# pagmerek/frave

Hardware: AMD Instinct MI355X
Metric: Mpixels/s encode (transform+quant) at 4096x4096 (higher is better)
Workload: dtype u8->i32

## Files before the change

### frave_amd/csrc/geometry.cpp

```cpp
#include "geometry.hpp"

#include <algorithm>
#include <climits>
#include <cstdlib>
#include <cstring>
#include <deque>

namespace fri {

namespace {

constexpr Int2 kLiterals[11] = {{0, 1}, {-1, 1}, {2, 0}, {-3, -1}, {5, -1}, {1, 3}, {-11, -1}, {9, -5}, {13, 7}, {-31, 3}, {5, -17}};

inline Int2 add(Int2 a, Int2 b) { return {a.x + b.x, a.y + b.y}; }
inline Int2 sub(Int2 a, Int2 b) { return {a.x - b.x, a.y - b.y}; }
inline Int2 neg(Int2 a) { return {-a.x, -a.y}; }
inline int floor_div(int a, int b) { return (a >= 0) ? a / b : -((-a + b - 1) / b); }
inline int pos_mod(int a, int m) {
    int r = a % m;
    return r < 0 ? r + m : r;
}

struct LatticeBasis {
    Int2 zl, zmd;
// ... 383 lines not shown
        for (size_t sh = 0; sh < n_wg; sh++) {
            const Tile &first = g.tiles[g.wg_tiles[sh]], &last = g.tiles[g.wg_tiles[sh + 1] - 1];
            g.max_wg_cells = std::max(g.max_wg_cells, last.cell_begin + last.cell_count - first.cell_begin);
            g.max_wg_tiles = std::max(g.max_wg_tiles, g.wg_tiles[sh + 1] - g.wg_tiles[sh]);
        }
    }
    if (tp.strided_shares && n_wg > 1) {
        std::vector<std::vector<int32_t>> dealt(n_wg);
        size_t next = 0;
        for (bool any = true; any && next < T;) {
            any = false;
            for (size_t sh = 0; sh < n_wg && next < T; sh++)
                if (dealt[sh].size() < (size_t)(g.wg_tiles[sh + 1] - g.wg_tiles[sh])) {
                    dealt[sh].push_back((int32_t)next++);
                    any = true;
                }
        }
        std::vector<Tile> tiles2;
        std::vector<TileCell> meta2;
        std::vector<int32_t> cells2;
        tiles2.reserve(T), meta2.reserve(F), cells2.reserve(F);
        g.max_wg_cells = 0;
        for (size_t sh = 0; sh < n_wg; sh++) {
            int32_t share_cells = 0;
            for (int32_t t_old : dealt[sh]) {
                Tile t = g.tiles[t_old];
                const int32_t begin = (int32_t)meta2.size();
                for (int32_t k = 0; k < t.cell_count; k++) {
                    meta2.push_back(g.tile_meta[t.cell_begin + k]);
                    cells2.push_back(g.tile_cells[t.cell_begin + k]);
                }
                t.cell_begin = begin;
                share_cells += t.cell_count;
                tiles2.push_back(t);
            }
            g.max_wg_cells = std::max(g.max_wg_cells, share_cells);
        }
        g.tiles.swap(tiles2);
        g.tile_meta.swap(meta2);
        g.tile_cells.swap(cells2);
    }
    {
        const size_t cells_target = (size_t)(tp.batch_share_tiles > 0 ? tp.batch_share_tiles : 4) * cells_per_tile;
        size_t merge = 1;
        while (merge * (size_t)g.cells_per_wg < cells_target && merge < n_wg) merge++;
        for (size_t sh = 0; sh < n_wg; sh += merge) g.wg_tiles_batch.push_back(g.wg_tiles[sh]);
        g.wg_tiles_batch.push_back(g.wg_tiles[n_wg]);
        for (size_t k = 0; k + 1 < g.wg_tiles_batch.size(); k++) g.max_wg_tiles_batch = std::max(g.max_wg_tiles_batch, g.wg_tiles_batch[k + 1] - g.wg_tiles_batch[k]);
    }
    int pitch = ((max_w * (int)channels + 15 + 15) / 16) * 16;
    while (((pitch / 4) % 32) != 8 && ((pitch / 4) % 32) != 24) pitch += 16;
    g.lds_pitch = pitch;
    g.lds_rows = max_r;
    return "";
}

void build_inverse_lists(Geometry &g, size_t max_bytes) {
    const StaticTables &st = static_tables();
    const int W = (int)g.width, H = (int)g.height, C = (int)g.channels;
    g.inv_lists.clear();
    g.inv_quads.clear();
    g.inv_dwords.clear();
    g.inv_parts.clear();
    g.inv_rect_bytes = 0;
    auto give_up = [&]() {
        g.inv_quads.clear();
        g.inv_dwords.clear();
        g.inv_parts.clear();
    };
    std::vector<InvTileLists> lists(g.tiles.size());
    std::vector<uint16_t> bitmap;
    for (size_t ti = 0; ti < g.tiles.size(); ti++) {
        const Tile &t = g.tiles[ti];
        const int a0 = (t.x_lo * C) & ~15;
        const int rq = ((t.x_lo + t.width_px) * C - 1 - a0) / 16 + 1;
        if (t.n_rows > 256 || rq > 64) return give_up();
        g.inv_rect_bytes = std::max(g.inv_rect_bytes, t.n_rows * rq * 16);
        bitmap.assign((size_t)t.n_rows * rq, 0);
        for (int c = 0; c < t.cell_count; c++) {
            const Int2 cen = g.centers[g.tile_cells[t.cell_begin + c]];
            for (int s2 = 0; s2 < kCell; s2++) {
                const int x = cen.x + st.leaf_off[s2].x, y = cen.y + st.leaf_off[s2].y;
                if (x < 0 || y < 0 || x >= W || y >= H) continue;
                for (int ch = 0; ch < C; ch++) {
                    const int col = x * C + ch - a0;
                    bitmap[(size_t)(y - t.y_lo) * rq + (col >> 4)] |= (uint16_t)(1u << (col & 15));
                }
            }
        }
        lists[ti].quad_begin = (uint32_t)g.inv_quads.size();
        lists[ti].dword_begin = (uint32_t)g.inv_dwords.size();
        lists[ti].part_begin = (uint32_t)g.inv_parts.size();
        for (int r = 0; r < t.n_rows; r++)
            for (int k = 0; k < rq; k++) {
                const uint16_t m = bitmap[(size_t)r * rq + k];
                if (m == 0xFFFFu) {
                    g.inv_quads.push_back((uint16_t)(r << 8 | k));
                } else if (m) {
                    for (int d = 0; d < 4; d++) {
                        const uint32_t nib = (m >> (4 * d)) & 15u;
                        if (nib == 15u)
                            g.inv_dwords.push_back((uint16_t)(r << 8 | (4 * k + d)));
                        else if (nib)
                            g.inv_parts.push_back((uint32_t)(r << 8 | (4 * k + d)) << 4 | nib);
                    }
                }
// ... 11 lines not shown
```

### frave_amd/csrc/k1_forward.hip

```cpp
#include "device_common.hpp"

namespace fri {
namespace {

constexpr int kFwdThreads = 256;
constexpr int kFwdWaves = kFwdThreads / 64;

constexpr int kMaxPairsPerWave = 2;
constexpr int kMaxItemsPerTile = 2 * kMaxPairsPerWave * kFwdWaves;
constexpr int kMaxChunksPerThread = 6;

struct FwdArgs {
    const uint8_t *pixels;
    size_t pixel_stride;
    int32_t *coefs;
    size_t coef_stride;
    const Tile *tiles;
    const TileCell *tile_meta;
    const int32_t *wg_tiles;
    uint32_t n_wg;
    int32_t width, height;
    uint32_t F;
    int32_t pitch;
    int32_t meta_off;
    int32_t buf_bytes;
    uint32_t cpr, cpr_magic;
    int32_t q_identity;
    int32_t ablate;
    unsigned long long *trace;
    unsigned long long *xcd_stat;
    QMatrix q;
};

__device__ __forceinline__ uint32_t pk_low(uint32_t l, uint32_t r, uint32_t x) { return __builtin_amdgcn_lerp(l, r, x >> 15); }
__device__ __forceinline__ void pk_pair(uint32_t l, uint32_t r, int &dA, int &dB, uint32_t &s) {
    s = pk_low(l, r, l - r);
    dA = (int)(l & 0xFFFFu) - (int)(r & 0xFFFFu);
    dB = (int)(l >> 16) - (int)(r >> 16);
}
__device__ __forceinline__ void unpack_x(uint32_t x, int &dA, int &dB) {
    dA = (int)(short)(x & 0xFFFFu);
    dB = (int)(x + 0x8000u) >> 16;
}

template <int J>
__device__ __forceinline__ uint32_t dpp_sibling(uint32_t v) {
    constexpr int ctrl = J == 0 ? 0xB1 : J == 1 ? 0x4E : J == 2 ? 0x141 : 0x140;
    return (uint32_t)__builtin_amdgcn_mov_dpp((int)v, ctrl, 0xF, 0xF, true);
}
template <int J>
__device__ __forceinline__ void pk_cross(int lane, int tz, uint32_t &s, uint32_t &vlow) {
    uint32_t x;
    if constexpr (J < 4) {
        const uint32_t other = dpp_sibling<J>(s);
        x = other - s;
        const uint32_t flip = ((lane >> J) & 1) ? 0u : 0x00010001u;
        s = __builtin_amdgcn_lerp(s, other, (x >> 15) ^ flip);
    } else {
        const uint2v w = J == 4 ? __builtin_amdgcn_permlane16_swap(s, s, false, false) : __builtin_amdgcn_permlane32_swap(s, s, false, false);
        x = w.x - w.y;
        s = pk_low(w.x, w.y, x);
    }
    if (tz == J) vlow = x;
}
template <int J>
__device__ __forceinline__ int xlane_or(int v) {
    if constexpr (J < 4) {
        return v | (int)dpp_sibling<J>((uint32_t)v);
    } else {
        const uint2v w = J == 4 ? __builtin_amdgcn_permlane16_swap((unsigned)v, (unsigned)v, false, false) : __builtin_amdgcn_permlane32_swap((unsigned)v, (unsigned)v, false, false);
        return (int)(w.x | w.y);
    }
}

__device__ __forceinline__ void fwd_wave_pk(const uint32_t (&leaf)[8], int lane, int (&rA)[8], int (&rB)[8]) {
    uint32_t s8[4], s7[2], s;
#pragma unroll
    for (int i = 0; i < 4; i++) pk_pair(leaf[2 * i], leaf[2 * i + 1], rA[i], rB[i], s8[i]);
#pragma unroll
    for (int i = 0; i < 2; i++) pk_pair(s8[2 * i], s8[2 * i + 1], rA[4 + i], rB[4 + i], s7[i]);
    pk_pair(s7[0], s7[1], rA[6], rB[6], s);
    const int tz = lane ? __builtin_ctz(lane) : 6;
    uint32_t vlow = 0;
    pk_cross<0>(lane, tz, s, vlow);
    pk_cross<1>(lane, tz, s, vlow);
    pk_cross<2>(lane, tz, s, vlow);
    pk_cross<3>(lane, tz, s, vlow);
    pk_cross<4>(lane, tz, s, vlow);
    pk_cross<5>(lane, tz, s, vlow);
    if (lane == 0) vlow = s;
    unpack_x((uint32_t)__shfl((int)vlow, low_source_lane(lane)), rA[7], rB[7]);
}

__device__ __forceinline__ uint32_t validity_tree_pk(uint32_t m, int lane) {
    const uint32_t v8 = (m | (m >> 1)) & 0x00550055u;
    const uint32_t v7 = (v8 | (v8 >> 2)) & 0x00110011u;
    int sv = (int)((v7 | (v7 >> 4)) & 0x00010001u);
    const uint32_t v6 = (uint32_t)sv;
    const int tz = lane ? __builtin_ctz(lane) : 6;
    int vlow = 0;
    sv = xlane_or<0>(sv); if (tz == 0) vlow = sv;
    sv = xlane_or<1>(sv); if (tz == 1) vlow = sv;
    sv = xlane_or<2>(sv); if (tz == 2) vlow = sv;
    sv = xlane_or<3>(sv); if (tz == 3) vlow = sv;
    sv = xlane_or<4>(sv); if (tz == 4) vlow = sv;
    sv = xlane_or<5>(sv); if (tz == 5) vlow = sv;
    if (lane == 0) vlow = sv;
    const uint32_t low = (uint32_t)__shfl(vlow, low_source_lane(lane));
    uint32_t out = (v8 & 0x00010001u) | ((v8 >> 1) & 0x00020002u) | ((v8 >> 2) & 0x00040004u) | ((v8 >> 3) & 0x00080008u);
    out |= ((v7 & 0x00010001u) << 4) | ((v7 & 0x00100010u) << 1);
    out |= (v6 << 6) | (low << 7);
    return out;
}

__device__ __forceinline__ int quant_one(int v, int heap_index, const FwdArgs &a) {
    return v == kNone ? v : v / a.q.q[quant_layer(heap_index)];
}

template <int HALF, bool MASKED, bool QID, bool NT, bool C16 = false>
__device__ __forceinline__ void store_item(int32_t *__restrict__ coefs, uint32_t elem_off, int lane, const int (&res)[8], uint32_t valid,
                                           const FwdArgs &a) {
    int v[8];
#pragma unroll
    for (int i = 0; i < 8; i++) {
        v[i] = res[i];
        if (MASKED && !((valid >> (16 * HALF + i)) & 1u)) v[i] = kNone;
    }
    if (!QID) {
#pragma unroll
        for (int i = 0; i < 4; i++) v[i] = quant_one(v[i], 256 + 4 * lane + i, a);
        v[4] = quant_one(v[4], 128 + 2 * lane, a);
        v[5] = quant_one(v[5], 128 + 2 * lane + 1, a);
        v[6] = quant_one(v[6], 64 + lane, a);
        v[7] = quant_one(v[7], lane, a);
    }
    int32_t *out = coefs + elem_off;
    if constexpr (C16) {
        int16_t *o16 = reinterpret_cast<int16_t *>(coefs) + elem_off;
        if (MASKED) {
#pragma unroll
            for (int i = 0; i < 8; i++) v[i] = v[i] == kNone ? 0 : v[i];
        }
        const uint32_t p0 = ((uint32_t)v[0] & 0xFFFFu) | ((uint32_t)v[1] << 16), p1 = ((uint32_t)v[2] & 0xFFFFu) | ((uint32_t)v[3] << 16);
        const uint32_t p2 = ((uint32_t)v[4] & 0xFFFFu) | ((uint32_t)v[5] << 16);
        *reinterpret_cast<i32x2 *>(o16 + 256 + 4 * lane) = i32x2{(int)p0, (int)p1};
        *reinterpret_cast<uint32_t *>(o16 + 128 + 2 * lane) = p2;
        o16[64 + lane] = (int16_t)v[6];
        o16[lane] = (int16_t)v[7];
        return;
    }
    if constexpr (NT) {
        __builtin_nontemporal_store(i32x4{v[0], v[1], v[2], v[3]}, reinterpret_cast<i32x4 *>(out + 256 + 4 * lane));
        __builtin_nontemporal_store(i32x2{v[4], v[5]}, reinterpret_cast<i32x2 *>(out + 128 + 2 * lane));
        __builtin_nontemporal_store(v[6], out + 64 + lane);
        __builtin_nontemporal_store(v[7], out + lane);
    } else {
        *reinterpret_cast<i32x4 *>(out + 256 + 4 * lane) = i32x4{v[0], v[1], v[2], v[3]};
        *reinterpret_cast<i32x2 *>(out + 128 + 2 * lane) = i32x2{v[4], v[5]};
        out[64 + lane] = v[6];
        out[lane] = v[7];
    }
// ... 124 lines not shown
    } else {
#pragma unroll
        for (int k = 0; k < 7; k++) g[k] = 0x80808080u;
    }
}
__device__ __forceinline__ uint32_t rct_leaf(uint32_t x, uint32_t g) { return (x + 0x01800180u - g) & 0x00FF00FFu; }

template <int DELTA>
__device__ __forceinline__ uint32_t shifted_window(uint32_t d0, uint32_t d1, uint32_t d2, uint32_t s) {
    return s + DELTA < 4u ? __builtin_amdgcn_alignbyte(d1, d0, s + DELTA) : __builtin_amdgcn_alignbyte(d2, d1, s + DELTA - 4u);
}
[[maybe_unused]] __device__ __forceinline__ void fetch_windows_ycc(int buf_off, const int (&rb)[3], uint32_t (&r)[7], uint32_t (&g)[7], uint32_t (&b)[7]) {
    const uint32_t b0 = (uint32_t)(buf_off + rb[0]), b1 = (uint32_t)(buf_off + rb[1] - 3), b2 = (uint32_t)(buf_off + rb[2] - 3);
    const LdsDwordPtr p0 = (LdsDwordPtr)(uintptr_t)(b0 & ~3u), p1 = (LdsDwordPtr)(uintptr_t)(b1 & ~3u), p2 = (LdsDwordPtr)(uintptr_t)(b2 & ~3u);
    const uint32_t d00 = p0[0], d01 = p0[1], d02 = p0[2];
    const uint32_t d10 = p1[0], d11 = p1[1], d12 = p1[2], d13 = p1[3];
    const uint32_t d20 = p2[0], d21 = p2[1], d22 = p2[2];
    const uint32_t s0 = b0 & 3u, s1 = b1 & 3u, s2 = b2 & 3u;
    r[0] = __builtin_amdgcn_alignbyte(d01, d00, s0), g[0] = shifted_window<1>(d00, d01, d02, s0), b[0] = shifted_window<2>(d00, d01, d02, s0);
    r[1] = __builtin_amdgcn_alignbyte(d02, d01, s0), g[1] = shifted_window<1>(d01, d02, d02, s0), b[1] = shifted_window<2>(d01, d02, d02, s0);
    r[2] = __builtin_amdgcn_alignbyte(d11, d10, s1), g[2] = shifted_window<1>(d10, d11, d12, s1), b[2] = shifted_window<2>(d10, d11, d12, s1);
    r[3] = __builtin_amdgcn_alignbyte(d12, d11, s1), g[3] = shifted_window<1>(d11, d12, d13, s1), b[3] = shifted_window<2>(d11, d12, d13, s1);
    r[4] = __builtin_amdgcn_alignbyte(d13, d12, s1), g[4] = shifted_window<1>(d12, d13, d13, s1), b[4] = shifted_window<2>(d12, d13, d13, s1);
    r[5] = __builtin_amdgcn_alignbyte(d21, d20, s2), g[5] = shifted_window<1>(d20, d21, d22, s2), b[5] = shifted_window<2>(d20, d21, d22, s2);
    r[6] = __builtin_amdgcn_alignbyte(d22, d21, s2), g[6] = shifted_window<1>(d21, d22, d22, s2), b[6] = shifted_window<2>(d21, d22, d22, s2);
}
struct YccWeights {
    int kr, kg, kb, bias;
};
[[maybe_unused]] __device__ __forceinline__ YccWeights ycc_weights(int plane) {
    if (plane == 0) return {19595, 38470, 7471, 32768};
    if (plane == 1) return {-11059, -21709, 32768, (128 << 16) + 32767};
    return {32768, -27439, -5329, (128 << 16) + 32767};
}
[[maybe_unused]] __device__ __forceinline__ uint32_t ycc_leaf(uint32_t r, uint32_t g, uint32_t b, const YccWeights &wa, const YccWeights &wb) {
    const int va = (__mul24(wa.kr, (int)(r & 0xFFFFu)) + __mul24(wa.kg, (int)(g & 0xFFFFu)) + __mul24(wa.kb, (int)(b & 0xFFFFu)) + wa.bias) >> 16;
    const int vb = (__mul24(wb.kr, (int)(r >> 16)) + __mul24(wb.kg, (int)(g >> 16)) + __mul24(wb.kb, (int)(b >> 16)) + wb.bias) >> 16;
    return (uint32_t)va | ((uint32_t)vb << 16);
}

template <int I>
__device__ __forceinline__ uint32_t pair_bytes(uint32_t a, uint32_t b) {
    return __builtin_amdgcn_perm(b, a, 0x0C000C00u | ((4u + I) << 16) | (unsigned)I);
}

struct ItemAddr {
    int rb[3];
    uint32_t leaf_mask;
    uint32_t elem_off;
};

__device__ __forceinline__ int rct_source(int ch) { return ch == 2 ? 0 : ch + 1; }

template <int C, bool FAST, bool RCT = false, bool YCC = false>
__device__ __forceinline__ ItemAddr item_addr(const FwdArgs &a, const Tile &t, const TileCell *meta, int it, int ldx, int ldy, int lane_rb, int buf_off,
                                               uint32_t sh_base, uint32_t wc16) {
    const int cl = it / C, plane = it - cl * C, ch = YCC ? 0 : RCT ? rct_source(plane) : plane;
    const TileCell m = meta[cl];
    ItemAddr r;
    r.elem_off = ((uint32_t)plane * a.F + (uint32_t)__builtin_amdgcn_readfirstlane(m.cell)) * kCell;
    const int x0 = m.cx + ldx, y0 = m.cy + ldy;
    const int col = __mul24(x0 - t.x_lo, C) + ch;
    if (FAST) {
        const int cell_base = (__builtin_amdgcn_readfirstlane(m.cy) - t.y_lo) * a.pitch + (__builtin_amdgcn_readfirstlane(m.cx) - t.x_lo) * C + ch + (int)(sh_base & 15u);
        r.rb[0] = cell_base + lane_rb + (C == 1 ? buf_off : 0);
        r.rb[1] = r.rb[0] + (C == 1 ? a.pitch - 1 : a.pitch);
        r.rb[2] = r.rb[0] + (C == 1 ? 2 * a.pitch - 1 : 2 * a.pitch);
    } else {
#pragma unroll
        for (int dy = 0; dy < 3; dy++) {
            const int y = y0 + dy;
            const uint32_t sh = (sh_base + __umul24((uint32_t)y & 15u, wc16)) & 15u;
            r.rb[dy] = __mul24(y - t.y_lo, a.pitch) + (int)sh + col + (C == 1 ? buf_off - (dy ? 1 : 0) : 0);
        }
    }
    r.leaf_mask = 0xFFu;
    if (__builtin_amdgcn_readfirstlane(m.interior) == 0) {
        r.leaf_mask = 0;
#pragma unroll
        for (int j = 0; j < 8; j++) {
            const int x = x0 + leaf_dx(j), y = y0 + leaf_dy(j);
            if (x >= 0 && y >= 0 && x < a.width && y < a.height) r.leaf_mask |= 1u << j;
        }
    }
    return r;
}

template <int C, bool EDGE, bool FAST, int NCH, bool QID, bool NT, bool MEASURE = false, bool C16 = false, bool RCT = false, bool YCC = false>
__global__ void __launch_bounds__(kFwdThreads) fwd_transform_quant_kernel(const FwdArgs a) {
    extern __shared__ __attribute__((aligned(16))) uint8_t lds[];
    if (ablate_flags(a.ablate) & 8) return;
    const int tid = threadIdx.x, lane = tid & 63;
    const int wave = __builtin_amdgcn_readfirstlane(tid >> 6);
    const uint32_t wg = xcd_contiguous_share(blockIdx.x, a.n_wg);
    const int tb = a.wg_tiles[wg], te = a.wg_tiles[wg + 1];
    trace_stamp(a.trace, wg, 0, tid);
    const unsigned long long t_entry = a.xcd_stat ? wall_clock64() : 0ull;
    uint8_t *junk = lds + 2 * a.buf_bytes;
    Tile *lds_tiles = reinterpret_cast<Tile *>(junk + 16 * kFwdThreads);
    if (tid < te - tb) lds_tiles[tid] = a.tiles[tb + tid];
    const uint8_t *img = a.pixels + (size_t)blockIdx.y * a.pixel_stride;
    int32_t *coefs = C16 ? reinterpret_cast<int32_t *>(reinterpret_cast<int16_t *>(a.coefs) + (size_t)blockIdx.y * a.coef_stride)
                         : a.coefs + (size_t)blockIdx.y * a.coef_stride;
    const int ldx = lane_dx(lane), ldy = lane_dy(lane);
    const int lane_rb = ldy * a.pitch + ldx * C;
    const uint32_t a16 = (uint32_t)reinterpret_cast<uintptr_t>(img);
    const uint32_t wc = (uint32_t)a.width * C, wc16 = wc & 15u;

    ChunkMap<NCH> cm;
#pragma unroll
    for (int c = 0; c < NCH; c++) {
        const uint32_t i = (uint32_t)tid + (uint32_t)c * kFwdThreads;
        const uint32_t r = a.cpr == 1 ? i : __umulhi(i, a.cpr_magic);
        cm.r[c] = r;
        cm.k16[c] = 16u * (i - r * a.cpr);
        cm.row_off[c] = r * wc;
    }

    u32x4 st[NCH + 1];
    Tile t = a.tiles[tb];
    stage_issue<C, EDGE, FAST, NCH>(a, t, img, tid, cm, st);
    stage_commit<NCH>(a, t, lds, junk, tid, st);
    __syncthreads();
    trace_stamp(a.trace, wg, 1, tid);

    for (int ti = tb; ti < te; ti++) {
        const uint8_t *cur = lds + ((ti - tb) & 1) * a.buf_bytes;
        const int buf_off = (int)(uint32_t)(uintptr_t)(const __attribute__((address_space(3))) uint8_t *)cur;
        uint8_t *nxt = lds + (((ti - tb) & 1) ^ 1) * a.buf_bytes;
        const bool more = ti + 1 < te;
        Tile tn = t;
        if (more) {
            const Tile &l = lds_tiles[ti + 1 - tb];
            tn.x_lo = __builtin_amdgcn_readfirstlane(l.x_lo);
            tn.y_lo = __builtin_amdgcn_readfirstlane(l.y_lo);
            tn.width_px = __builtin_amdgcn_readfirstlane(l.width_px);
            tn.n_rows = __builtin_amdgcn_readfirstlane(l.n_rows);
            tn.cell_begin = __builtin_amdgcn_readfirstlane(l.cell_begin);
            tn.cell_count = __builtin_amdgcn_readfirstlane(l.cell_count);
            stage_issue<C, EDGE, FAST, NCH>(a, tn, img, tid, cm, st);
        }

        if constexpr (C == 1) __builtin_amdgcn_s_setprio(3);
        const TileCell *meta = reinterpret_cast<const TileCell *>(cur + a.meta_off);
        const int n_items = (ablate_flags(a.ablate) & 2) ? 0 : t.cell_count * C;
        const uint32_t sh_base = a16 + (uint32_t)t.x_lo * C;
        int resA[kMaxPairsPerWave][8], resB[kMaxPairsPerWave][8];
        uint32_t offA[kMaxPairsPerWave], offB[kMaxPairsPerWave], valid[kMaxPairsPerWave];
#pragma unroll
        for (int c = 0; c < kMaxPairsPerWave; c++) {
            const int itA = 2 * (wave + kFwdWaves * c);
            offA[c] = offB[c] = 0;
            valid[c] = 0xFFFFFFFFu;
            if (itA < n_items) {
                const int itB = itA + 1 < n_items ? itA + 1 : itA;
                const ItemAddr A = item_addr<C, FAST, RCT, YCC>(a, t, meta, itA, ldx, ldy, lane_rb, buf_off, sh_base, wc16);
                const ItemAddr B = item_addr<C, FAST, RCT, YCC>(a, t, meta, itB, ldx, ldy, lane_rb, buf_off, sh_base, wc16);
                offA[c] = A.elem_off;
                offB[c] = B.elem_off;
                uint32_t leaf[8];
                if constexpr (C == 1) {
                    uint32_t wA[3], wB[3];
                    fetch_windows(A.rb, wA);
                    fetch_windows(B.rb, wB);
                    if ((A.leaf_mask & B.leaf_mask) != 0xFFu) {
                        mask_windows(A.leaf_mask, wA);
                        mask_windows(B.leaf_mask, wB);
                    }
                    leaf[0] = pair_bytes<0>(wA[0], wB[0]);
                    leaf[1] = pair_bytes<1>(wA[1], wB[1]);
                    leaf[2] = pair_bytes<0>(wA[1], wB[1]);
                    leaf[3] = pair_bytes<0>(wA[2], wB[2]);
                    leaf[4] = pair_bytes<2>(wA[0], wB[0]);
                    leaf[5] = pair_bytes<3>(wA[1], wB[1]);
                    leaf[6] = pair_bytes<2>(wA[1], wB[1]);
                    leaf[7] = pair_bytes<2>(wA[2], wB[2]);
                } else if constexpr (YCC) {
                    uint32_t rA[7], gA[7], bA[7], rB[7], gB[7], bB[7];
                    fetch_windows_ycc(buf_off, A.rb, rA, gA, bA);
                    fetch_windows_ycc(buf_off, B.rb, rB, gB, bB);
                    const YccWeights kA = ycc_weights(itA % 3), kB = ycc_weights(itB % 3);
                    leaf[0] = ycc_leaf(pair_bytes<0>(rA[0], rB[0]), pair_bytes<0>(gA[0], gB[0]), pair_bytes<0>(bA[0], bB[0]), kA, kB);
                    leaf[4] = ycc_leaf(pair_bytes<2>(rA[1], rB[1]), pair_bytes<2>(gA[1], gB[1]), pair_bytes<2>(bA[1], bB[1]), kA, kB);
                    leaf[2] = ycc_leaf(pair_bytes<0>(rA[2], rB[2]), pair_bytes<0>(gA[2], gB[2]), pair_bytes<0>(bA[2], bB[2]), kA, kB);
                    leaf[1] = ycc_leaf(pair_bytes<3>(rA[2], rB[2]), pair_bytes<3>(gA[2], gB[2]), pair_bytes<3>(bA[2], bB[2]), kA, kB);
                    leaf[6] = ycc_leaf(pair_bytes<2>(rA[3], rB[3]), pair_bytes<2>(gA[3], gB[3]), pair_bytes<2>(bA[3], bB[3]), kA, kB);
                    leaf[5] = ycc_leaf(pair_bytes<1>(rA[4], rB[4]), pair_bytes<1>(gA[4], gB[4]), pair_bytes<1>(bA[4], bB[4]), kA, kB);
                    leaf[3] = ycc_leaf(pair_bytes<0>(rA[5], rB[5]), pair_bytes<0>(gA[5], gB[5]), pair_bytes<0>(bA[5], bB[5]), kA, kB);
                    leaf[7] = ycc_leaf(pair_bytes<2>(rA[6], rB[6]), pair_bytes<2>(gA[6], gB[6]), pair_bytes<2>(bA[6], bB[6]), kA, kB);
                    if ((A.leaf_mask & B.leaf_mask) != 0xFFu) {
#pragma unroll
                        for (int j = 0; j < 8; j++) {
                            if (!((A.leaf_mask >> j) & 1u)) leaf[j] &= 0xFFFF0000u;
                            if (!((B.leaf_mask >> j) & 1u)) leaf[j] &= 0x0000FFFFu;
                        }
                    }
                } else {
                    uint32_t wA[7], wB[7];
                    fetch_windows_rgb(buf_off, A.rb, wA);
                    fetch_windows_rgb(buf_off, B.rb, wB);
                    leaf[0] = pair_bytes<0>(wA[0], wB[0]);
                    leaf[4] = pair_bytes<2>(wA[1], wB[1]);
                    leaf[2] = pair_bytes<0>(wA[2], wB[2]);
                    leaf[1] = pair_bytes<3>(wA[2], wB[2]);
                    leaf[6] = pair_bytes<2>(wA[3], wB[3]);
                    leaf[5] = pair_bytes<1>(wA[4], wB[4]);
                    leaf[3] = pair_bytes<0>(wA[5], wB[5]);
                    leaf[7] = pair_bytes<2>(wA[6], wB[6]);
                    if constexpr (RCT) {
                        const int chA = rct_source(itA % 3), chB = rct_source(itB % 3);
                        uint32_t gA[7], gB[7];
                        fetch_g_windows_item(buf_off, A.rb, chA, gA);
                        fetch_g_windows_item(buf_off, B.rb, chB, gB);
                        leaf[0] = rct_leaf(leaf[0], pair_bytes<0>(gA[0], gB[0]));
                        leaf[4] = rct_leaf(leaf[4], pair_bytes<2>(gA[1], gB[1]));
                        leaf[2] = rct_leaf(leaf[2], pair_bytes<0>(gA[2], gB[2]));
                        leaf[1] = rct_leaf(leaf[1], pair_bytes<3>(gA[2], gB[2]));
                        leaf[6] = rct_leaf(leaf[6], pair_bytes<2>(gA[3], gB[3]));
                        leaf[5] = rct_leaf(leaf[5], pair_bytes<1>(gA[4], gB[4]));
                        leaf[3] = rct_leaf(leaf[3], pair_bytes<0>(gA[5], gB[5]));
                        leaf[7] = rct_leaf(leaf[7], pair_bytes<2>(gA[6], gB[6]));
                    }
                    if ((A.leaf_mask & B.leaf_mask) != 0xFFu) {
#pragma unroll
                        for (int j = 0; j < 8; j++) {
                            if (!((A.leaf_mask >> j) & 1u)) leaf[j] &= 0xFFFF0000u;
                            if (!((B.leaf_mask >> j) & 1u)) leaf[j] &= 0x0000FFFFu;
                        }
                    }
                }
                fwd_wave_pk(leaf, lane, resA[c], resB[c]);
                if constexpr (C == 1) {
                    if (c == 0)
                        __builtin_amdgcn_s_setprio(2);
                    else
                        __builtin_amdgcn_s_setprio(1);
                }
                if (__builtin_amdgcn_readfirstlane(meta[itA / C].interior & meta[itB / C].interior) == 0)
                    valid[c] = validity_tree_pk(A.leaf_mask | (B.leaf_mask << 16), lane);
            }
        }
        if (more) stage_commit<NCH>(a, tn, nxt, junk, tid, st);
        if constexpr (C == 1) __builtin_amdgcn_s_setprio(0);
#pragma unroll
        for (int c = 0; c < kMaxPairsPerWave; c++) {
            const int itA = 2 * (wave + kFwdWaves * c);
            if (itA < n_items) {
                bool go = !(ablate_flags(a.ablate) & 4);
                if (!go) go = (resA[c][0] ^ resA[c][1] ^ resA[c][2] ^ resA[c][3] ^ resA[c][4] ^ resA[c][5] ^ resA[c][6] ^ resA[c][7] ^ resB[c][0] ^ resB[c][1] ^ resB[c][2] ^ resB[c][3] ^
                               resB[c][4] ^ resB[c][5] ^ resB[c][6] ^ resB[c][7]) == 0x12345678;
                if (go) {
                    if (__builtin_amdgcn_readfirstlane(valid[c] == 0xFFFFFFFFu ? 1 : 0) && __all(valid[c] == 0xFFFFFFFFu)) {
                        store_item<0, false, QID, NT, C16>(coefs, offA[c], lane, resA[c], valid[c], a);
                        if (itA + 1 < n_items) store_item<1, false, QID, NT, C16>(coefs, offB[c], lane, resB[c], valid[c], a);
                    } else {
                        store_item<0, true, QID, NT, C16>(coefs, offA[c], lane, resA[c], valid[c], a);
                        if (itA + 1 < n_items) store_item<1, true, QID, NT, C16>(coefs, offB[c], lane, resB[c], valid[c], a);
                    }
                }
            }
        }
        trace_stamp(a.trace, wg, 2 + ti - tb, tid);
        lds_barrier();
        t = tn;
    }
    trace_exit(a.trace, wg, tid);
    if (a.xcd_stat && tid == 0) {
        const uint32_t xcc = __builtin_amdgcn_s_getreg((3 << 11) | 20) & 7u;
        (void)__hip_atomic_fetch_add(a.xcd_stat + 2 * xcc, wall_clock64() - t_entry, __ATOMIC_RELAXED, __HIP_MEMORY_SCOPE_AGENT);
        (void)__hip_atomic_fetch_add(a.xcd_stat + 2 * xcc + 1, 1ull, __ATOMIC_RELAXED, __HIP_MEMORY_SCOPE_AGENT);
    }
}


}

const void *pick_forward_ycbcr(bool edge, bool fast, bool small, bool qid, bool plain, bool measure, bool c16);
#ifndef FRI_K1_YCBCR_INSTANCES

static size_t fwd_meta_offset(const DevicePlan &p) { return ((size_t)p.lds_pitch * p.lds_rows + 15) & ~(size_t)15; }
static size_t fwd_buf_bytes(const DevicePlan &p) { return fwd_meta_offset(p) + (size_t)p.max_tile_cells * sizeof(TileCell); }
size_t fwd_lds_bytes(const DevicePlan &p) { return 2 * fwd_buf_bytes(p) + 16 * kFwdThreads + (size_t)p.max_wg_tiles * sizeof(Tile); }
static size_t fwd_chunks(const DevicePlan &p) { return (size_t)p.lds_rows * (p.lds_pitch / 16); }

bool device_footprint_matches(const StaticTables &st) {
    for (int l = 0; l < 64; l++)
        for (int j = 0; j < 8; j++) {
            const Int2 o = st.leaf_off[8 * l + j];
            if (o.x != lane_dx(l) + leaf_dx(j) || o.y != lane_dy(l) + leaf_dy(j)) return false;
        }
    return true;
}

bool fwd_plan_fits(const DevicePlan &p) {
    return fwd_chunks(p) <= (size_t)kMaxChunksPerThread * kFwdThreads &&
           (size_t)p.max_tile_cells * p.channels <= (size_t)kMaxItemsPerTile && p.max_tile_cells <= kFwdThreads &&
           p.max_wg_tiles <= kFwdThreads && fwd_lds_bytes(p) <= 160 * 1024;
}

hipError_t launch_fwd_transform_quant(const DevicePlan &p, uint32_t n_images, const uint8_t *pixels, size_t pixel_stride, int32_t *coefs,
                                      size_t coef_stride, const QMatrix &q, hipStream_t stream, bool cached_stores, int16_t *coefs16) {
    if (!fwd_plan_fits(p)) return hipErrorInvalidConfiguration;
    const bool plain = p.k1_cached_stores >= 0 ? p.k1_cached_stores > 0 : cached_stores;
    FwdArgs a{};
    a.pixels = pixels;
    a.pixel_stride = pixel_stride;
    a.coefs = coefs16 ? reinterpret_cast<int32_t *>(coefs16) : coefs;
    a.coef_stride = coef_stride;
    a.tiles = p.tiles;
    a.tile_meta = p.tile_meta;
    const bool batch = n_images >= 8 && p.n_wg_batch > 0 && p.n_wg_batch < p.n_wg && p.k1_batch_shares;
    a.wg_tiles = batch ? p.wg_tiles_batch : p.wg_tiles;
    a.n_wg = batch ? p.n_wg_batch : p.n_wg;
    a.width = p.width;
    a.height = p.height;
    a.F = p.F;
    a.pitch = p.lds_pitch;
    a.meta_off = (int32_t)fwd_meta_offset(p);
    a.buf_bytes = (int32_t)fwd_buf_bytes(p);
    a.cpr = (uint32_t)p.lds_pitch / 16u;
    a.cpr_magic = (uint32_t)(((1ull << 32) + a.cpr - 1) / a.cpr);
    a.q = q;
    a.q_identity = 1;
    for (int i = 0; i <= 9; i++) a.q_identity &= (q.q[i] == 1);
    a.ablate = p.k1_ablate;
    a.trace = p.trace;
    a.xcd_stat = p.k1_xcd_stat;
    const size_t lds = fwd_lds_bytes(p);
    const dim3 grid(a.n_wg, n_images), block(kFwdThreads);
    const size_t img_bytes = (size_t)p.width * p.height * p.channels;
    const bool edge = (reinterpret_cast<uintptr_t>(pixels) & 15) || (img_bytes & 15) || (n_images > 1 && (pixel_stride & 15));
    const bool fast = !edge && (((size_t)p.width * p.channels) & 15) == 0;
    const bool small = fwd_chunks(p) <= 4 * (size_t)kFwdThreads;
    const bool rct = p.rct && p.channels == 3;
    const bool ycc = p.ycc && p.channels == 3;
    void (*kern)(FwdArgs);
#define FRI_PICK_T(CH, E, FA, N, QI, R) (plain ? fwd_transform_quant_kernel<CH, E, FA, N, QI, false, false, false, R> : fwd_transform_quant_kernel<CH, E, FA, N, QI, true, false, false, R>)
#define FRI_PICK_Q(CH, E, FA, N, R) (a.q_identity ? FRI_PICK_T(CH, E, FA, N, true, R) : FRI_PICK_T(CH, E, FA, N, false, R))
#define FRI_PICK_N(CH, E, FA, R) (small ? FRI_PICK_Q(CH, E, FA, 4, R) : FRI_PICK_Q(CH, E, FA, kMaxChunksPerThread, R))
#define FRI_PICK(CH, R) (edge ? FRI_PICK_N(CH, true, false, R) : fast ? FRI_PICK_N(CH, false, true, R) : FRI_PICK_N(CH, false, false, R))
    kern = p.channels == 1 ? FRI_PICK(1, false) : rct ? FRI_PICK(3, true) : FRI_PICK(3, false);
    if (p.k1_measuring && !edge && !plain && a.q_identity) {
#define FRI_PICK_M(CH, R) (fast ? (small ? fwd_transform_quant_kernel<CH, false, true, 4, true, true, true, false, R> : fwd_transform_quant_kernel<CH, false, true, kMaxChunksPerThread, true, true, true, false, R>) \
                                : (small ? fwd_transform_quant_kernel<CH, false, false, 4, true, true, true, false, R> : fwd_transform_quant_kernel<CH, false, false, kMaxChunksPerThread, true, true, true, false, R>))
        kern = p.channels == 1 ? FRI_PICK_M(1, false) : rct ? FRI_PICK_M(3, true) : FRI_PICK_M(3, false);
#undef FRI_PICK_M
    }
    if (coefs16) {
#define FRI_PICK_C(CH, E, FA, N, R) (a.q_identity ? fwd_transform_quant_kernel<CH, E, FA, N, true, false, false, true, R> : fwd_transform_quant_kernel<CH, E, FA, N, false, false, false, true, R>)
#define FRI_PICK_CN(CH, E, FA, R) (small ? FRI_PICK_C(CH, E, FA, 4, R) : FRI_PICK_C(CH, E, FA, kMaxChunksPerThread, R))
#define FRI_PICK_CC(CH, R) (edge ? FRI_PICK_CN(CH, true, false, R) : fast ? FRI_PICK_CN(CH, false, true, R) : FRI_PICK_CN(CH, false, false, R))
        kern = p.channels == 1 ? FRI_PICK_CC(1, false) : rct ? FRI_PICK_CC(3, true) : FRI_PICK_CC(3, false);
#undef FRI_PICK_CC
#undef FRI_PICK_CN
#undef FRI_PICK_C
    }
#undef FRI_PICK
#undef FRI_PICK_N
#undef FRI_PICK_Q
#undef FRI_PICK_T
    if (ycc) kern = reinterpret_cast<void (*)(FwdArgs)>(const_cast<void *>(pick_forward_ycbcr(edge, fast, small, a.q_identity != 0, plain, p.k1_measuring && !edge && !plain && a.q_identity, coefs16 != nullptr)));
    if (lds > 48 * 1024) {
        hipError_t e = hipFuncSetAttribute(reinterpret_cast<const void *>(kern), hipFuncAttributeMaxDynamicSharedMemorySize, (int)lds);
        if (e != hipSuccess) return e;
    }
    (void)hipGetLastError();
    hipLaunchKernelGGL(kern, grid, block, lds, stream, a);
    return hipGetLastError();
}
#endif

}
```

### frave_amd/csrc/k1_ycbcr.hip

```cpp
#define FRI_K1_YCBCR_INSTANCES 1
#include "k1_forward.hip"

namespace fri {

template <bool E, bool FA, int N>
static const void *pick_ycc_n(bool qid, bool plain, bool measure, bool c16) {
    if (c16)
        return qid ? reinterpret_cast<const void *>(fwd_transform_quant_kernel<3, E, FA, N, true, false, false, true, false, true>)
                   : reinterpret_cast<const void *>(fwd_transform_quant_kernel<3, E, FA, N, false, false, false, true, false, true>);
    if constexpr (!E) {
        if (measure) return reinterpret_cast<const void *>(fwd_transform_quant_kernel<3, false, FA, N, true, true, true, false, false, true>);
    }
    if (qid)
        return plain ? reinterpret_cast<const void *>(fwd_transform_quant_kernel<3, E, FA, N, true, false, false, false, false, true>)
                     : reinterpret_cast<const void *>(fwd_transform_quant_kernel<3, E, FA, N, true, true, false, false, false, true>);
    return plain ? reinterpret_cast<const void *>(fwd_transform_quant_kernel<3, E, FA, N, false, false, false, false, false, true>)
                 : reinterpret_cast<const void *>(fwd_transform_quant_kernel<3, E, FA, N, false, true, false, false, false, true>);
}
template <bool E, bool FA>
static const void *pick_ycc(bool small, bool qid, bool plain, bool measure, bool c16) {
    return small ? pick_ycc_n<E, FA, 4>(qid, plain, measure, c16) : pick_ycc_n<E, FA, kMaxChunksPerThread>(qid, plain, measure, c16);
}
const void *pick_forward_ycbcr(bool edge, bool fast, bool small, bool qid, bool plain, bool measure, bool c16) {
    return edge ? pick_ycc<true, false>(small, qid, plain, measure, c16) : fast ? pick_ycc<false, true>(small, qid, plain, measure, c16)
                                                                                : pick_ycc<false, false>(small, qid, plain, measure, c16);
}

}
```

Baseline: 903,000.

## Hoist per-lane constants, specialize pair count, defer boundary masks in forward kernel

```diff
diff --git a/frave_amd/csrc/geometry.cpp b/frave_amd/csrc/geometry.cpp
--- a/frave_amd/csrc/geometry.cpp
+++ b/frave_amd/csrc/geometry.cpp
@@ -459,6 +459,9 @@
     while (((pitch / 4) % 32) != 8 && ((pitch / 4) % 32) != 24) pitch += 16;
     g.lds_pitch = pitch;
     g.lds_rows = max_r;
+    for (const std::vector<int32_t> *w : {&g.wg_tiles, &g.wg_tiles_batch})
+        for (size_t sh = 0; sh + 1 < w->size(); sh++)
+            if ((*w)[sh + 1] <= (*w)[sh]) return "forward tiling: a workgroup share without a tile";
     return "";
 }
 
diff --git a/frave_amd/csrc/k1_forward.hip b/frave_amd/csrc/k1_forward.hip
--- a/frave_amd/csrc/k1_forward.hip
+++ b/frave_amd/csrc/k1_forward.hip
@@ -8,6 +8,7 @@
 
 constexpr int kMaxPairsPerWave = 2;
 constexpr int kMaxItemsPerTile = 2 * kMaxPairsPerWave * kFwdWaves;
+constexpr int kItemsOnePair = 2 * kFwdWaves;
 constexpr int kMaxChunksPerThread = 6;
 
 struct FwdArgs {
@@ -48,20 +49,37 @@
     constexpr int ctrl = J == 0 ? 0xB1 : J == 1 ? 0x4E : J == 2 ? 0x141 : 0x140;
     return (uint32_t)__builtin_amdgcn_mov_dpp((int)v, ctrl, 0xF, 0xF, true);
 }
+struct LaneConst {
+    uint32_t flip[4];
+    bool keep[6];
+    bool root;
+    int low_src;
+};
+__device__ __forceinline__ LaneConst lane_const(int lane) {
+    LaneConst lc;
+    const int tz = lane ? __builtin_ctz(lane) : 6;
+#pragma unroll
+    for (int j = 0; j < 4; j++) lc.flip[j] = ((lane >> j) & 1) ? 0u : 0x00010001u;
+#pragma unroll
+    for (int j = 0; j < 6; j++) lc.keep[j] = tz == j;
+    lc.root = lane == 0;
+    const int l1 = lane | (lane == 0 ? 1 : 0), lv = 31 - __clz(l1), m = l1 - (1 << lv);
+    lc.low_src = lane ? (2 * m + 1) << (5 - lv) : 0;
+    return lc;
+}
 template <int J>
-__device__ __forceinline__ void pk_cross(int lane, int tz, uint32_t &s, uint32_t &vlow) {
+__device__ __forceinline__ void pk_cross(const LaneConst &lc, uint32_t &s, uint32_t &vlow) {
     uint32_t x;
     if constexpr (J < 4) {
         const uint32_t other = dpp_sibling<J>(s);
         x = other - s;
-        const uint32_t flip = ((lane >> J) & 1) ? 0u : 0x00010001u;
-        s = __builtin_amdgcn_lerp(s, other, (x >> 15) ^ flip);
+        s = __builtin_amdgcn_lerp(s, other, (x >> 15) ^ lc.flip[J]);
     } else {
         const uint2v w = J == 4 ? __builtin_amdgcn_permlane16_swap(s, s, false, false) : __builtin_amdgcn_permlane32_swap(s, s, false, false);
         x = w.x - w.y;
         s = pk_low(w.x, w.y, x);
     }
-    if (tz == J) vlow = x;
+    if (lc.keep[J]) vlow = x;
 }
 template <int J>
 __device__ __forceinline__ int xlane_or(int v) {
@@ -73,40 +91,38 @@
     }
 }
 
-__device__ __forceinline__ void fwd_wave_pk(const uint32_t (&leaf)[8], int lane, int (&rA)[8], int (&rB)[8]) {
+__device__ __forceinline__ void fwd_wave_pk(const uint32_t (&leaf)[8], const LaneConst &lc, int (&rA)[8], int (&rB)[8]) {
     uint32_t s8[4], s7[2], s;
 #pragma unroll
     for (int i = 0; i < 4; i++) pk_pair(leaf[2 * i], leaf[2 * i + 1], rA[i], rB[i], s8[i]);
 #pragma unroll
     for (int i = 0; i < 2; i++) pk_pair(s8[2 * i], s8[2 * i + 1], rA[4 + i], rB[4 + i], s7[i]);
     pk_pair(s7[0], s7[1], rA[6], rB[6], s);
-    const int tz = lane ? __builtin_ctz(lane) : 6;
     uint32_t vlow = 0;
-    pk_cross<0>(lane, tz, s, vlow);
-    pk_cross<1>(lane, tz, s, vlow);
-    pk_cross<2>(lane, tz, s, vlow);
-    pk_cross<3>(lane, tz, s, vlow);
-    pk_cross<4>(lane, tz, s, vlow);
-    pk_cross<5>(lane, tz, s, vlow);
-    if (lane == 0) vlow = s;
-    unpack_x((uint32_t)__shfl((int)vlow, low_source_lane(lane)), rA[7], rB[7]);
-}
-
-__device__ __forceinline__ uint32_t validity_tree_pk(uint32_t m, int lane) {
+    pk_cross<0>(lc, s, vlow);
+    pk_cross<1>(lc, s, vlow);
+    pk_cross<2>(lc, s, vlow);
+    pk_cross<3>(lc, s, vlow);
+    pk_cross<4>(lc, s, vlow);
+    pk_cross<5>(lc, s, vlow);
+    if (lc.root) vlow = s;
+    unpack_x((uint32_t)__shfl((int)vlow, lc.low_src), rA[7], rB[7]);
+}
+
+__device__ __forceinline__ uint32_t validity_tree_pk(uint32_t m, const LaneConst &lc) {
     const uint32_t v8 = (m | (m >> 1)) & 0x00550055u;
     const uint32_t v7 = (v8 | (v8 >> 2)) & 0x00110011u;
     int sv = (int)((v7 | (v7 >> 4)) & 0x00010001u);
     const uint32_t v6 = (uint32_t)sv;
-    const int tz = lane ? __builtin_ctz(lane) : 6;
     int vlow = 0;
-    sv = xlane_or<0>(sv); if (tz == 0) vlow = sv;
-    sv = xlane_or<1>(sv); if (tz == 1) vlow = sv;
-    sv = xlane_or<2>(sv); if (tz == 2) vlow = sv;
-    sv = xlane_or<3>(sv); if (tz == 3) vlow = sv;
-    sv = xlane_or<4>(sv); if (tz == 4) vlow = sv;
-    sv = xlane_or<5>(sv); if (tz == 5) vlow = sv;
-    if (lane == 0) vlow = sv;
-    const uint32_t low = (uint32_t)__shfl(vlow, low_source_lane(lane));
+    sv = xlane_or<0>(sv); if (lc.keep[0]) vlow = sv;
+    sv = xlane_or<1>(sv); if (lc.keep[1]) vlow = sv;
+    sv = xlane_or<2>(sv); if (lc.keep[2]) vlow = sv;
+    sv = xlane_or<3>(sv); if (lc.keep[3]) vlow = sv;
+    sv = xlane_or<4>(sv); if (lc.keep[4]) vlow = sv;
+    sv = xlane_or<5>(sv); if (lc.keep[5]) vlow = sv;
+    if (lc.root) vlow = sv;
+    const uint32_t low = (uint32_t)__shfl(vlow, lc.low_src);
     uint32_t out = (v8 & 0x00010001u) | ((v8 >> 1) & 0x00020002u) | ((v8 >> 2) & 0x00040004u) | ((v8 >> 3) & 0x00080008u);
     out |= ((v7 & 0x00010001u) << 4) | ((v7 & 0x00100010u) << 1);
     out |= (v6 << 6) | (low << 7);
@@ -337,17 +353,34 @@
 
 __device__ __forceinline__ int rct_source(int ch) { return ch == 2 ? 0 : ch + 1; }
 
+__device__ __forceinline__ TileCell read_cell(const TileCell *meta, int cl) {
+    const TileCell m = meta[cl];
+    return TileCell{__builtin_amdgcn_readfirstlane(m.cx), __builtin_amdgcn_readfirstlane(m.cy), __builtin_amdgcn_readfirstlane(m.cell),
+                    __builtin_amdgcn_readfirstlane(m.interior)};
+}
+
+__device__ __forceinline__ uint32_t boundary_leaf_mask(const FwdArgs &a, const TileCell &m, int ldx, int ldy) {
+    if (m.interior) return 0xFFu;
+    const int x0 = m.cx + ldx, y0 = m.cy + ldy;
+    uint32_t mask = 0;
+#pragma unroll
+    for (int j = 0; j < 8; j++) {
+        const int x = x0 + leaf_dx(j), y = y0 + leaf_dy(j);
+        if (x >= 0 && y >= 0 && x < a.width && y < a.height) mask |= 1u << j;
+    }
+    return mask;
+}
+
 template <int C, bool FAST, bool RCT = false, bool YCC = false>
-__device__ __forceinline__ ItemAddr item_addr(const FwdArgs &a, const Tile &t, const TileCell *meta, int it, int ldx, int ldy, int lane_rb, int buf_off,
+__device__ __forceinline__ ItemAddr item_addr(const FwdArgs &a, const Tile &t, const TileCell &m, int it, int ldx, int ldy, int lane_rb, int buf_off,
                                                uint32_t sh_base, uint32_t wc16) {
     const int cl = it / C, plane = it - cl * C, ch = YCC ? 0 : RCT ? rct_source(plane) : plane;
-    const TileCell m = meta[cl];
     ItemAddr r;
-    r.elem_off = ((uint32_t)plane * a.F + (uint32_t)__builtin_amdgcn_readfirstlane(m.cell)) * kCell;
+    r.elem_off = ((uint32_t)plane * a.F + (uint32_t)m.cell) * kCell;
     const int x0 = m.cx + ldx, y0 = m.cy + ldy;
     const int col = __mul24(x0 - t.x_lo, C) + ch;
     if (FAST) {
-        const int cell_base = (__builtin_amdgcn_readfirstlane(m.cy) - t.y_lo) * a.pitch + (__builtin_amdgcn_readfirstlane(m.cx) - t.x_lo) * C + ch + (int)(sh_base & 15u);
+        const int cell_base = (m.cy - t.y_lo) * a.pitch + (m.cx - t.x_lo) * C + ch + (int)(sh_base & 15u);
         r.rb[0] = cell_base + lane_rb + (C == 1 ? buf_off : 0);
         r.rb[1] = r.rb[0] + (C == 1 ? a.pitch - 1 : a.pitch);
         r.rb[2] = r.rb[0] + (C == 1 ? 2 * a.pitch - 1 : 2 * a.pitch);
@@ -360,18 +393,10 @@
         }
     }
     r.leaf_mask = 0xFFu;
-    if (__builtin_amdgcn_readfirstlane(m.interior) == 0) {
-        r.leaf_mask = 0;
-#pragma unroll
-        for (int j = 0; j < 8; j++) {
-            const int x = x0 + leaf_dx(j), y = y0 + leaf_dy(j);
-            if (x >= 0 && y >= 0 && x < a.width && y < a.height) r.leaf_mask |= 1u << j;
-        }
-    }
     return r;
 }
 
-template <int C, bool EDGE, bool FAST, int NCH, bool QID, bool NT, bool MEASURE = false, bool C16 = false, bool RCT = false, bool YCC = false>
+template <int C, bool EDGE, bool FAST, int NCH, int NP, bool QID, bool NT, bool MEASURE = false, bool C16 = false, bool RCT = false, bool YCC = false>
 __global__ void __launch_bounds__(kFwdThreads) fwd_transform_quant_kernel(const FwdArgs a) {
     extern __shared__ __attribute__((aligned(16))) uint8_t lds[];
     if (ablate_flags(a.ablate) & 8) return;
@@ -379,11 +404,11 @@
     const int wave = __builtin_amdgcn_readfirstlane(tid >> 6);
     const uint32_t wg = xcd_contiguous_share(blockIdx.x, a.n_wg);
     const int tb = a.wg_tiles[wg], te = a.wg_tiles[wg + 1];
+    Tile t = a.tiles[tb];
     trace_stamp(a.trace, wg, 0, tid);
     const unsigned long long t_entry = a.xcd_stat ? wall_clock64() : 0ull;
     uint8_t *junk = lds + 2 * a.buf_bytes;
     Tile *lds_tiles = reinterpret_cast<Tile *>(junk + 16 * kFwdThreads);
-    if (tid < te - tb) lds_tiles[tid] = a.tiles[tb + tid];
     const uint8_t *img = a.pixels + (size_t)blockIdx.y * a.pixel_stride;
     int32_t *coefs = C16 ? reinterpret_cast<int32_t *>(reinterpret_cast<int16_t *>(a.coefs) + (size_t)blockIdx.y * a.coef_stride)
                          : a.coefs + (size_t)blockIdx.y * a.coef_stride;
@@ -403,13 +428,22 @@
     }
 
     u32x4 st[NCH + 1];
-    Tile t = a.tiles[tb];
     stage_issue<C, EDGE, FAST, NCH>(a, t, img, tid, cm, st);
+    const int my_tile = min(tid, te - tb - 1);
+    const int32_t *tile_src = reinterpret_cast<const int32_t *>(a.tiles + tb + my_tile);
+    int32_t mine[6];
+#pragma unroll
+    for (int i = 0; i < 6; i++) mine[i] = tile_src[i];
+    const LaneConst lc = lane_const(lane);
+    __builtin_amdgcn_sched_barrier(0);
     stage_commit<NCH>(a, t, lds, junk, tid, st);
+#pragma unroll
+    for (int i = 0; i < 6; i++) reinterpret_cast<int32_t *>(lds_tiles + my_tile)[i] = mine[i];
     __syncthreads();
     trace_stamp(a.trace, wg, 1, tid);
 
-    for (int ti = tb; ti < te; ti++) {
+    int ti = tb;
+    do {
         const uint8_t *cur = lds + ((ti - tb) & 1) * a.buf_bytes;
         const int buf_off = (int)(uint32_t)(uintptr_t)(const __attribute__((address_space(3))) uint8_t *)cur;
         uint8_t *nxt = lds + (((ti - tb) & 1) ^ 1) * a.buf_bytes;
@@ -430,17 +464,24 @@
         const TileCell *meta = reinterpret_cast<const TileCell *>(cur + a.meta_off);
         const int n_items = (ablate_flags(a.ablate) & 2) ? 0 : t.cell_count * C;
         const uint32_t sh_base = a16 + (uint32_t)t.x_lo * C;
-        int resA[kMaxPairsPerWave][8], resB[kMaxPairsPerWave][8];
-        uint32_t offA[kMaxPairsPerWave], offB[kMaxPairsPerWave], valid[kMaxPairsPerWave];
-#pragma unroll
-        for (int c = 0; c < kMaxPairsPerWave; c++) {
+        static_assert(NP >= 1 && NP <= kMaxPairsPerWave, "a wave carries one or two pairs per tile");
+        int resA[NP][8], resB[NP][8];
+        uint32_t offA[NP], offB[NP], valid[NP];
+#pragma unroll
+        for (int c = 0; c < NP; c++) {
             const int itA = 2 * (wave + kFwdWaves * c);
             offA[c] = offB[c] = 0;
             valid[c] = 0xFFFFFFFFu;
             if (itA < n_items) {
                 const int itB = itA + 1 < n_items ? itA + 1 : itA;
-                const ItemAddr A = item_addr<C, FAST, RCT, YCC>(a, t, meta, itA, ldx, ldy, lane_rb, buf_off, sh_base, wc16);
-                const ItemAddr B = item_addr<C, FAST, RCT, YCC>(a, t, meta, itB, ldx, ldy, lane_rb, buf_off, sh_base, wc16);
+                const TileCell mA = read_cell(meta, itA / C), mB = read_cell(meta, itB / C);
+                ItemAddr A = item_addr<C, FAST, RCT, YCC>(a, t, mA, itA, ldx, ldy, lane_rb, buf_off, sh_base, wc16);
+                ItemAddr B = item_addr<C, FAST, RCT, YCC>(a, t, mB, itB, ldx, ldy, lane_rb, buf_off, sh_base, wc16);
+                const bool boundary = (mA.interior & mB.interior) == 0;
+                if (boundary) {
+                    A.leaf_mask = boundary_leaf_mask(a, mA, ldx, ldy);
+                    B.leaf_mask = boundary_leaf_mask(a, mB, ldx, ldy);
+                }
                 offA[c] = A.elem_off;
                 offB[c] = B.elem_off;
                 uint32_t leaf[8];
@@ -448,7 +489,7 @@
                     uint32_t wA[3], wB[3];
                     fetch_windows(A.rb, wA);
                     fetch_windows(B.rb, wB);
-                    if ((A.leaf_mask & B.leaf_mask) != 0xFFu) {
+                    if (boundary && (A.leaf_mask & B.leaf_mask) != 0xFFu) {
                         mask_windows(A.leaf_mask, wA);
                         mask_windows(B.leaf_mask, wB);
                     }
@@ -473,7 +514,7 @@
                     leaf[5] = ycc_leaf(pair_bytes<1>(rA[4], rB[4]), pair_bytes<1>(gA[4], gB[4]), pair_bytes<1>(bA[4], bB[4]), kA, kB);
                     leaf[3] = ycc_leaf(pair_bytes<0>(rA[5], rB[5]), pair_bytes<0>(gA[5], gB[5]), pair_bytes<0>(bA[5], bB[5]), kA, kB);
                     leaf[7] = ycc_leaf(pair_bytes<2>(rA[6], rB[6]), pair_bytes<2>(gA[6], gB[6]), pair_bytes<2>(bA[6], bB[6]), kA, kB);
-                    if ((A.leaf_mask & B.leaf_mask) != 0xFFu) {
+                    if (boundary && (A.leaf_mask & B.leaf_mask) != 0xFFu) {
 #pragma unroll
                         for (int j = 0; j < 8; j++) {
                             if (!((A.leaf_mask >> j) & 1u)) leaf[j] &= 0xFFFF0000u;
@@ -506,7 +547,7 @@
                         leaf[3] = rct_leaf(leaf[3], pair_bytes<0>(gA[5], gB[5]));
                         leaf[7] = rct_leaf(leaf[7], pair_bytes<2>(gA[6], gB[6]));
                     }
-                    if ((A.leaf_mask & B.leaf_mask) != 0xFFu) {
+                    if (boundary && (A.leaf_mask & B.leaf_mask) != 0xFFu) {
 #pragma unroll
                         for (int j = 0; j < 8; j++) {
                             if (!((A.leaf_mask >> j) & 1u)) leaf[j] &= 0xFFFF0000u;
@@ -514,21 +555,20 @@
                         }
                     }
                 }
-                fwd_wave_pk(leaf, lane, resA[c], resB[c]);
+                fwd_wave_pk(leaf, lc, resA[c], resB[c]);
                 if constexpr (C == 1) {
                     if (c == 0)
                         __builtin_amdgcn_s_setprio(2);
                     else
                         __builtin_amdgcn_s_setprio(1);
                 }
-                if (__builtin_amdgcn_readfirstlane(meta[itA / C].interior & meta[itB / C].interior) == 0)
-                    valid[c] = validity_tree_pk(A.leaf_mask | (B.leaf_mask << 16), lane);
+                if (boundary) valid[c] = validity_tree_pk(A.leaf_mask | (B.leaf_mask << 16), lc);
             }
         }
         if (more) stage_commit<NCH>(a, tn, nxt, junk, tid, st);
         if constexpr (C == 1) __builtin_amdgcn_s_setprio(0);
 #pragma unroll
-        for (int c = 0; c < kMaxPairsPerWave; c++) {
+        for (int c = 0; c < NP; c++) {
             const int itA = 2 * (wave + kFwdWaves * c);
             if (itA < n_items) {
                 bool go = !(ablate_flags(a.ablate) & 4);
@@ -548,7 +588,7 @@
         trace_stamp(a.trace, wg, 2 + ti - tb, tid);
         lds_barrier();
         t = tn;
-    }
+    } while (++ti < te);
     trace_exit(a.trace, wg, tid);
     if (a.xcd_stat && tid == 0) {
         const uint32_t xcc = __builtin_amdgcn_s_getreg((3 << 11) | 20) & 7u;
@@ -619,23 +659,24 @@
     const bool small = fwd_chunks(p) <= 4 * (size_t)kFwdThreads;
     const bool rct = p.rct && p.channels == 3;
     const bool ycc = p.ycc && p.channels == 3;
+    const bool one_pair = p.channels == 1 && p.max_tile_cells <= kItemsOnePair;
     void (*kern)(FwdArgs);
-#define FRI_PICK_T(CH, E, FA, N, QI, R) (plain ? fwd_transform_quant_kernel<CH, E, FA, N, QI, false, false, false, R> : fwd_transform_quant_kernel<CH, E, FA, N, QI, true, false, false, R>)
-#define FRI_PICK_Q(CH, E, FA, N, R) (a.q_identity ? FRI_PICK_T(CH, E, FA, N, true, R) : FRI_PICK_T(CH, E, FA, N, false, R))
-#define FRI_PICK_N(CH, E, FA, R) (small ? FRI_PICK_Q(CH, E, FA, 4, R) : FRI_PICK_Q(CH, E, FA, kMaxChunksPerThread, R))
-#define FRI_PICK(CH, R) (edge ? FRI_PICK_N(CH, true, false, R) : fast ? FRI_PICK_N(CH, false, true, R) : FRI_PICK_N(CH, false, false, R))
-    kern = p.channels == 1 ? FRI_PICK(1, false) : rct ? FRI_PICK(3, true) : FRI_PICK(3, false);
+#define FRI_PICK_T(CH, E, FA, N, P, QI, R) (plain ? fwd_transform_quant_kernel<CH, E, FA, N, P, QI, false, false, false, R> : fwd_transform_quant_kernel<CH, E, FA, N, P, QI, true, false, false, R>)
+#define FRI_PICK_Q(CH, E, FA, N, P, R) (a.q_identity ? FRI_PICK_T(CH, E, FA, N, P, true, R) : FRI_PICK_T(CH, E, FA, N, P, false, R))
+#define FRI_PICK_N(CH, E, FA, P, R) (small ? FRI_PICK_Q(CH, E, FA, 4, P, R) : FRI_PICK_Q(CH, E, FA, kMaxChunksPerThread, P, R))
+#define FRI_PICK(CH, P, R) (edge ? FRI_PICK_N(CH, true, false, P, R) : fast ? FRI_PICK_N(CH, false, true, P, R) : FRI_PICK_N(CH, false, false, P, R))
+    kern = p.channels == 1 ? (one_pair ? FRI_PICK(1, 1, false) : FRI_PICK(1, 2, false)) : rct ? FRI_PICK(3, 2, true) : FRI_PICK(3, 2, false);
     if (p.k1_measuring && !edge && !plain && a.q_identity) {
-#define FRI_PICK_M(CH, R) (fast ? (small ? fwd_transform_quant_kernel<CH, false, true, 4, true, true, true, false, R> : fwd_transform_quant_kernel<CH, false, true, kMaxChunksPerThread, true, true, true, false, R>) \
-                                : (small ? fwd_transform_quant_kernel<CH, false, false, 4, true, true, true, false, R> : fwd_transform_quant_kernel<CH, false, false, kMaxChunksPerThread, true, true, true, false, R>))
-        kern = p.channels == 1 ? FRI_PICK_M(1, false) : rct ? FRI_PICK_M(3, true) : FRI_PICK_M(3, false);
+#define FRI_PICK_M(CH, P, R) (fast ? (small ? fwd_transform_quant_kernel<CH, false, true, 4, P, true, true, true, false, R> : fwd_transform_quant_kernel<CH, false, true, kMaxChunksPerThread, P, true, true, true, false, R>) \
+                                   : (small ? fwd_transform_quant_kernel<CH, false, false, 4, P, true, true, true, false, R> : fwd_transform_quant_kernel<CH, false, false, kMaxChunksPerThread, P, true, true, true, false, R>))
+        kern = p.channels == 1 ? (one_pair ? FRI_PICK_M(1, 1, false) : FRI_PICK_M(1, 2, false)) : rct ? FRI_PICK_M(3, 2, true) : FRI_PICK_M(3, 2, false);
 #undef FRI_PICK_M
     }
     if (coefs16) {
-#define FRI_PICK_C(CH, E, FA, N, R) (a.q_identity ? fwd_transform_quant_kernel<CH, E, FA, N, true, false, false, true, R> : fwd_transform_quant_kernel<CH, E, FA, N, false, false, false, true, R>)
-#define FRI_PICK_CN(CH, E, FA, R) (small ? FRI_PICK_C(CH, E, FA, 4, R) : FRI_PICK_C(CH, E, FA, kMaxChunksPerThread, R))
-#define FRI_PICK_CC(CH, R) (edge ? FRI_PICK_CN(CH, true, false, R) : fast ? FRI_PICK_CN(CH, false, true, R) : FRI_PICK_CN(CH, false, false, R))
-        kern = p.channels == 1 ? FRI_PICK_CC(1, false) : rct ? FRI_PICK_CC(3, true) : FRI_PICK_CC(3, false);
+#define FRI_PICK_C(CH, E, FA, N, P, R) (a.q_identity ? fwd_transform_quant_kernel<CH, E, FA, N, P, true, false, false, true, R> : fwd_transform_quant_kernel<CH, E, FA, N, P, false, false, false, true, R>)
+#define FRI_PICK_CN(CH, E, FA, P, R) (small ? FRI_PICK_C(CH, E, FA, 4, P, R) : FRI_PICK_C(CH, E, FA, kMaxChunksPerThread, P, R))
+#define FRI_PICK_CC(CH, P, R) (edge ? FRI_PICK_CN(CH, true, false, P, R) : fast ? FRI_PICK_CN(CH, false, true, P, R) : FRI_PICK_CN(CH, false, false, P, R))
+        kern = p.channels == 1 ? (one_pair ? FRI_PICK_CC(1, 1, false) : FRI_PICK_CC(1, 2, false)) : rct ? FRI_PICK_CC(3, 2, true) : FRI_PICK_CC(3, 2, false);
 #undef FRI_PICK_CC
 #undef FRI_PICK_CN
 #undef FRI_PICK_C
diff --git a/frave_amd/csrc/k1_ycbcr.hip b/frave_amd/csrc/k1_ycbcr.hip
--- a/frave_amd/csrc/k1_ycbcr.hip
+++ b/frave_amd/csrc/k1_ycbcr.hip
@@ -6,16 +6,16 @@
 template <bool E, bool FA, int N>
 static const void *pick_ycc_n(bool qid, bool plain, bool measure, bool c16) {
     if (c16)
-        return qid ? reinterpret_cast<const void *>(fwd_transform_quant_kernel<3, E, FA, N, true, false, false, true, false, true>)
-                   : reinterpret_cast<const void *>(fwd_transform_quant_kernel<3, E, FA, N, false, false, false, true, false, true>);
+        return qid ? reinterpret_cast<const void *>(fwd_transform_quant_kernel<3, E, FA, N, kMaxPairsPerWave, true, false, false, true, false, true>)
+                   : reinterpret_cast<const void *>(fwd_transform_quant_kernel<3, E, FA, N, kMaxPairsPerWave, false, false, false, true, false, true>);
     if constexpr (!E) {
-        if (measure) return reinterpret_cast<const void *>(fwd_transform_quant_kernel<3, false, FA, N, true, true, true, false, false, true>);
+        if (measure) return reinterpret_cast<const void *>(fwd_transform_quant_kernel<3, false, FA, N, kMaxPairsPerWave, true, true, true, false, false, true>);
     }
     if (qid)
-        return plain ? reinterpret_cast<const void *>(fwd_transform_quant_kernel<3, E, FA, N, true, false, false, false, false, true>)
-                     : reinterpret_cast<const void *>(fwd_transform_quant_kernel<3, E, FA, N, true, true, false, false, false, true>);
-    return plain ? reinterpret_cast<const void *>(fwd_transform_quant_kernel<3, E, FA, N, false, false, false, false, false, true>)
-                 : reinterpret_cast<const void *>(fwd_transform_quant_kernel<3, E, FA, N, false, true, false, false, false, true>);
+        return plain ? reinterpret_cast<const void *>(fwd_transform_quant_kernel<3, E, FA, N, kMaxPairsPerWave, true, false, false, false, false, true>)
+                     : reinterpret_cast<const void *>(fwd_transform_quant_kernel<3, E, FA, N, kMaxPairsPerWave, true, true, false, false, false, true>);
+    return plain ? reinterpret_cast<const void *>(fwd_transform_quant_kernel<3, E, FA, N, kMaxPairsPerWave, false, false, false, false, false, true>)
+                 : reinterpret_cast<const void *>(fwd_transform_quant_kernel<3, E, FA, N, kMaxPairsPerWave, false, true, false, false, false, true>);
 }
 template <bool E, bool FA>
 static const void *pick_ycc(bool small, bool qid, bool plain, bool measure, bool c16) {
```

New measurement: 922,600, median of 6. 1.02x the previous value.
